# SegoleneMartin/transductive-CLIP

Hardware: AMD Instinct MI355X
Metric: transductive tasks/sec (75-query EM-Dirichlet) (higher is better)
Workload: dtype f32

## Files before the change

transductive-clip_amd/csrc/tclip_kernels.hip:

```cpp
#include <hip/hip_runtime.h>
#include <stdint.h>
#include <stdio.h>
#include <stdlib.h>
#include <string.h>

#include <algorithm>
#include <mutex>
#include <utility>
#include <vector>

#include "../../include/tclip.h"
#include "tclip_device.h"
#include "tclip_pk.h"
#include "tclip_selftest_inputs.h"

namespace tclip {

constexpr int kG64MinK = 897;

__global__ void k_log_features(const float* __restrict__ x, float* __restrict__ out, size_t n, int32_t* __restrict__ nonfinite) {
    bool bad = false;
    for (size_t i = (size_t)blockIdx.x * blockDim.x + threadIdx.x; i < n; i += (size_t)gridDim.x * blockDim.x) {
        const float v = log_f32(x[i] + kEpsF);
        out[i] = v;
// ... 976 lines not shown
        pending = st;
    }
    if (E / 2 > 0) finish(E / 2 - 1, pending);
    if (E & 1) {
        constexpr int e = E - 1;
        const float a = beta[e];
        const int i = (int)(slot[e >> 1] & 0xffffu);
        const float nb = mm_update_algebra(a, y_of(e), psi_s, my1[i], my0[i]);
        const bool ok = elem_of<E, G>(e, lane) < K;
        if (measure && ok) {
            const double df = (double)nb - (double)a;
            num += df * df;
            den += (double)a * (double)a;
        }
        beta[e] = ok ? nb : 0.0f;
    }
}

__device__ __forceinline__ void wave_lds_handoff() {
    __builtin_amdgcn_fence(__ATOMIC_RELEASE, "wavefront");
    __builtin_amdgcn_wave_barrier();
    __builtin_amdgcn_fence(__ATOMIC_ACQUIRE, "wavefront");
}

template <int E>
struct SplitPlacement {
    uint32_t slot[(E + 1) / 2];
    int nA, nB, nC;
    bool valid;
    int sorts;
};

template <int E, int G, int KC>
__device__ __forceinline__ void split_place(const float (&beta)[E], int K, int lane, float* my0, SplitPlacement<E>& pl) {
    constexpr int kFirstRagged = first_ragged_register<E, G, KC>();
    int nA = 0, nC = 0, nV = kFirstRagged * 64;
#pragma unroll
    for (int e = 0; e < E; e++) {
        float x1 = beta[e] + 1.0f;
        asm volatile("" : "+v"(x1));
        unsigned long long mA = __builtin_amdgcn_ballot_w64(x1 < 2.3f), mC = __builtin_amdgcn_ballot_w64(x1 >= 10.0f);
        if (e >= kFirstRagged) {
            const bool in_row = elem_of<E, G>(e, lane) < K;
            const unsigned long long mv = __builtin_amdgcn_ballot_w64(in_row);
            mA &= mv;
            mC &= mv;
            nV += __popcll(mv);
        }
        nA += __popcll(mA);
        nC += __popcll(mC);
    }
    const int nB = nV - nA - nC;
    int cA = 0, cB = nA, cC = nA + nB;
#pragma unroll
    for (int e = 0; e < E; e++) {
        float x1 = beta[e] + 1.0f;
        asm volatile("" : "+v"(x1));
        const bool lt = x1 < 2.3f, ge = x1 >= 10.0f;
        unsigned long long mA = __builtin_amdgcn_ballot_w64(lt), mC = __builtin_amdgcn_ballot_w64(ge);
        unsigned long long mB = ~(mA | mC);
        bool in_row = true;
        if (e >= kFirstRagged) {
            in_row = elem_of<E, G>(e, lane) < K;
            const unsigned long long mv = __builtin_amdgcn_ballot_w64(in_row);
            mA &= mv;
            mC &= mv;
            mB &= mv;
        }
        const int iA = (int)__builtin_amdgcn_mbcnt_hi((unsigned)(mA >> 32), __builtin_amdgcn_mbcnt_lo((unsigned)mA, (unsigned)cA));
        const int iB = (int)__builtin_amdgcn_mbcnt_hi((unsigned)(mB >> 32), __builtin_amdgcn_mbcnt_lo((unsigned)mB, (unsigned)cB));
        const int iC = (int)__builtin_amdgcn_mbcnt_hi((unsigned)(mC >> 32), __builtin_amdgcn_mbcnt_lo((unsigned)mC, (unsigned)cC));
        int idx = lt ? iA : iB;
        idx = ge ? iC : idx;
        if (e >= kFirstRagged) {
            idx = in_row ? idx : 0;
            if (in_row) my0[idx] = x1;
        } else {
            my0[idx] = x1;
        }
        if (e & 1) pl.slot[e >> 1] |= (uint32_t)idx << 16;
        else pl.slot[e >> 1] = (uint32_t)idx;
        cA += __popcll(mA);
        cB += __popcll(mB);
        cC += __popcll(mC);
    }
    pl.nA = nA;
    pl.nB = nB;
    pl.nC = nC;
}

template <int E, int G, int KC>
__device__ __forceinline__ void split_scatter(const float (&beta)[E], int K, int lane, float* my0, const SplitPlacement<E>& pl) {
    constexpr int kFirstRagged = first_ragged_register<E, G, KC>();
#pragma unroll
    for (int e = 0; e < E; e++) {
        const float x1 = beta[e] + 1.0f;
        const int idx = (e & 1) ? (int)(pl.slot[e >> 1] >> 16) : (int)(pl.slot[e >> 1] & 0xffffu);
        if (e >= kFirstRagged) {
            if (elem_of<E, G>(e, lane) < K) my0[idx] = x1;
        } else {
            my0[idx] = x1;
        }
    }
}

template <int E, int G, int KC = 0>
__device__ __forceinline__ void mm_iterate_wave_split(float (&beta)[E], const RowY<E, G, kSplitYRegsMaxE>& yv, int K, int lane, bool active,
                                                      const LogTabEntry* tab, float* my0, float* my1, bool measure,
                                                      double& num, double& den, SplitPlacement<E>& pl, bool keep_placement) {
    const int lane64 = threadIdx.x & 63;
    float s = 16.0f;
    bool in_domain = true;
    if (active) {
        s = row_sum_torch<E, G, KC>(beta, K, lane);
        in_domain = lane != 0 || (fast_range_f32(s) && s <= 0x1p40f);
        uint32_t largest = 0u;
#pragma unroll
        for (int e = 0; e < E; e++) largest = max(largest, f32_bits(beta[e]));
        in_domain = in_domain & mm_fast_domain_of_max_bits(largest);
    }
    s = __shfl(s, 0, G);
    if (__builtin_expect(!__all(in_domain), 0)) {
        if (active) {
            const float psi_s = digamma_f32(s);
#pragma unroll
            for (int e = 0; e < E; e++) {
                const float nb = mm_update_generic(beta[e], yv.get(e), psi_s);
                const bool ok = elem_of<E, G>(e, lane) < K;
                if (measure && ok) {
                    const double df = (double)nb - (double)beta[e];
                    num += df * df;
                    den += (double)beta[e] * (double)beta[e];
                }
                beta[e] = ok ? nb : 0.0f;
            }
        }
        pl.valid = false;
        return;
    }
    constexpr int kFirstRagged = first_ragged_register<E, G, KC>();
    int32_t smallest = 0x7f800000;
#pragma unroll
    for (int e = 0; e < E; e++) {
        int32_t bits = (int32_t)f32_bits(beta[e]);
        if (e >= kFirstRagged) bits = elem_of<E, G>(e, lane) < K ? bits : 0x7f800000;
        smallest = bits < smallest ? bits : smallest;
    }
    const bool tiny = __builtin_amdgcn_ballot_w64(smallest <= (int32_t)0x2d2febffu) != 0ull;
    const float psi_s = digamma_pos_f32(s, tab);
    bool sort_now = !(keep_placement && pl.valid);
    for (;;) {
        if (sort_now) {
            split_place<E, G, KC>(beta, K, lane, my0, pl);
            pl.sorts++;
        } else split_scatter<E, G, KC>(beta, K, lane, my0, pl);
        const int nA = pl.nA, nB = pl.nB, nC = pl.nC;
        wave_lds_handoff();
        bool misplaced = false;
        int jA = 0;
        for (; jA + 64 < nA; jA += 128) {
            const int j = jA;
            const int i0 = j + lane64, i1 = min(i0 + 64, nA - 1);
            const f2 x{my0[i0], my0[i1]};
            if (!sort_now && __builtin_amdgcn_ballot_w64(!(fmaxf(x.x, x.y) < 2.3f)) != 0ull) { misplaced = true; break; }
            f2 xr = x, acc = pk(0.0f);
#pragma unroll
            for (int k = 0; k < 8; k++) {
                acc = acc - pk_rcp_rn(xr);
                xr = xr + pk(1.0f);
            }
            const f2 m{below10_f32(xr.x), below10_f32(xr.y)};
            acc = pk_fma(-m, pk_rcp_rn(xr), acc);
            xr = xr + m;
            const f2 psi = pk_digamma_after_rec(xr, acc, tab);
            const f2 lg = pk_lgamma_sleef_1_23(x);
            my0[i0] = lg.x;
            my1[i0] = psi.x;
            my0[i1] = lg.y;
            my1[i1] = psi.y;
        }
        for (; !misplaced && jA < nA; jA += 64) {
            const int i = min(jA + lane64, nA - 1);
            const float x = my0[i];
            if (!sort_now && __builtin_amdgcn_ballot_w64(!(x < 2.3f)) != 0ull) { misplaced = true; break; }
            float xr = x, acc = 0.0f;
#pragma unroll
            for (int k = 0; k < 8; k++) {
                acc = acc - rcp_rn_f32(xr);
                xr = xr + 1.0f;
            }
            const float m = below10_f32(xr);
            acc = __builtin_fmaf(-m, rcp_rn_f32(xr), acc);
            xr = xr + m;
            const float psi = digamma_after_rec_ge10<false>(xr, acc, tab);
            bool sure;
            float lg = lgamma_sleef_1_23_f64(x, sure);
            if (__builtin_expect(__builtin_amdgcn_ballot_w64(!sure) != 0ull, 0)) lg = sure ? lg : lgamma_sleef_05_23(x);
            my0[i] = lg;
            my1[i] = psi;
        }
        auto pass_b = [&](int i) -> bool {
            const float x = my0[i];
            if (!sort_now && __builtin_amdgcn_ballot_w64(!(x >= 2.3f)) != 0ull) return true;
            float xr = x, acc = 0.0f;
#pragma unroll
            for (int k = 0; k < 8; k++) {
                const float m = below10_f32(xr);
                acc = __builtin_fmaf(-m, rcp_rn_f32(xr), acc);
                xr += m;
            }
            const float psi = digamma_after_rec_ge10<false>(xr, acc, tab);
            const float lg = lgamma_big_dense(x);
            my0[i] = lg;
            my1[i] = psi;
            return false;
        };
        const int tB = nB & 63, tC = nC & 63;
        const bool merged = tB > 0 && tC > 0 && tB + tC <= 64;
        const int endB = merged ? nB - tB : nB, endC = merged ? nC - tC : nC;
        for (int j = 0; !misplaced && j < endB; j += 64) misplaced = pass_b(nA + min(j + lane64, endB - 1));
        if (merged && !misplaced) {
            const int l = min(lane64, tB + tC - 1);
            misplaced = pass_b(l < tB ? nA + endB + l : nA + nB + endC + (l - tB));
        }
        for (int j = 0; !misplaced && j < endC; j += 64) {
            const int i = nA + nB + min(j + lane64, endC - 1);
            const float x = my0[i];
            if (!sort_now && __builtin_amdgcn_ballot_w64(!(x >= 10.0f)) != 0ull) { misplaced = true; break; }
            const float psi = digamma_after_rec_ge10<true>(x, 0.0f, tab);
            const float lg = lgamma_gt7_dense(x);
            my0[i] = lg;
            my1[i] = psi;
        }
        if (!misplaced) break;
        sort_now = true;
        wave_lds_handoff();
    }
    pl.valid = true;
    wave_lds_handoff();
    if (__builtin_expect(measure, 0)) {
        if (tiny) split_apply_updates<E, G, true, true>(beta, yv, K, lane, psi_s, my0, my1, pl.slot, num, den);
        else split_apply_updates<E, G, false, true>(beta, yv, K, lane, psi_s, my0, my1, pl.slot, num, den);
    } else if (__builtin_expect(tiny, 0)) split_apply_updates<E, G, true, false>(beta, yv, K, lane, psi_s, my0, my1, pl.slot, num, den);
    else split_apply_updates<E, G, false, false>(beta, yv, K, lane, psi_s, my0, my1, pl.slot, num, den);
    wave_lds_handoff();
}

template <int E, int G, int KC = 0>
__global__ __launch_bounds__(64, (E > 16 ? kMMWavesLarge : kMMWavesSmall)) void k_mm_split(MMArgs a) {
    static_assert(E <= kSplitMaxE, "LDS: two words per element");
    __shared__ LogTabEntry tab[16];
    __shared__ float plane0[64 * E];
    __shared__ float plane1[64 * E];
    load_log_table(tab);
    const int lane = threadIdx.x & (G - 1);
    const int group = threadIdx.x / G;
    constexpr int kRows = 64 / G;
    const int n = *a.n_rows;
    const int K = KC > 0 ? KC : a.K;
    for (int first = blockIdx.x * kRows; first < n; first += gridDim.x * kRows) {
        const int i = first + group;
        int row = i < n ? a.rows[i] : 0;
        if constexpr (G == 64) row = __builtin_amdgcn_readfirstlane(row);
        const bool active = i < n && !a.stop[row / a.rows_per_batch];
        if (!__any(active)) continue;
        float beta[E];
        RowY<E, G, kSplitYRegsMaxE> yv;
        double num = 0.0, den = 0.0;
        yv.load(a.y + (size_t)row * K, lane, K);
#pragma unroll
        for (int e = 0; e < E; e++) {
            const int d = elem_of<E, G>(e, lane);
            beta[e] = (active && d < K) ? a.alpha[(size_t)row * K + d] : 0.0f;
        }
        SplitPlacement<E> pl;
        pl.valid = false;
        pl.sorts = 0;
        for (int l = a.l0; l <= a.l1; l++)
            mm_iterate_wave_split<E, G, KC>(beta, yv, K, lane, active, tab, plane0, plane1, a.has_check && l == a.l1, num, den, pl,
                                            a.keep_placement != 0);
        if (a.work_counter && (threadIdx.x & 63) == 0) {
            atomicAdd(a.work_counter + 1, (unsigned long long)(a.l1 - a.l0 + 1));
            atomicAdd(a.work_counter + 2, (unsigned long long)pl.sorts);
        }
        if (!active) continue;
#pragma unroll
        for (int e = 0; e < E; e++) {
            const int d = elem_of<E, G>(e, lane);
            if (d < K) a.alpha[(size_t)row * K + d] = beta[e];
        }
        if (a.work_counter && lane == 0)
            atomicAdd(a.work_counter, (unsigned long long)K * (unsigned long long)(a.l1 - a.l0 + 1));
        if (a.has_check) {
            const double sn = group_sum_f64_g<G>(num), sd = group_sum_f64_g<G>(den);
            if (lane == 0) {
                a.rowpart[2 * (size_t)row] = sn;
                a.rowpart[2 * (size_t)row + 1] = sd;
            }
        }
    }
}

constexpr int kReuseQueue = 768;
struct ReuseState {
    int nS, nL;
    bool full;
    int evaluated;
};

template <int E, int G, bool kTiny, bool kMeasure>
__device__ __forceinline__ void reuse_apply_updates(float (&beta)[E], const RowY<E, G, kSplitYRegsMaxE>& yv, int K, int lane, float psi_s,
                                                    float* my0, const float* my1, uint16_t* q, int cap, ReuseState& rs,
                                                    double& num, double& den) {
    constexpr bool measure = kMeasure;
    constexpr bool kYLocal = !RowY<E, G, kSplitYRegsMaxE>::kInRegs;
    float yl[kYLocal ? E : 1];
    if constexpr (kYLocal) yv.fetch_all(yl);
    auto y_of = [&](int e) { if constexpr (kYLocal) return yl[e]; else return yv.get(e); };
    const int n_full = full_registers<E, G>(K);
    const int lane64 = threadIdx.x & 63;
    float* h0 = my0 + lane64;
    const float* h1 = my1 + lane64;
    int cS = 0, cL = 0;
    auto note = [&](int e, float a, float nb) {
        const float xo = a + 1.0f, xn = nb + 1.0f;
        const bool dirty = xn != xo, small = xn < 2.3f;
        const unsigned long long mD = __builtin_amdgcn_ballot_w64(dirty), mSm = __builtin_amdgcn_ballot_w64(small);
        const unsigned long long mS = mD & mSm, mL = mD & ~mSm;
        const int rank = lanes_below(mS);
        if (dirty) h0[64 * e] = xn;
        uint16_t* qs = q + cS;
        if (dirty && small && rank < cap - cS) qs[rank] = (uint16_t)(64 * e + lane64);
        if (__builtin_expect(mL != 0ull, 0)) {
            const int rankL = lanes_below(mL);
            if (dirty && !small && rankL < cap - cL) q[cap - 1 - cL - rankL] = (uint16_t)(64 * e + lane64);
        }
        cS += __popcll(mS);
        cL += __popcll(mL);
    };
    auto finish = [&](int p, const PkUpdateStage& st) {
        const int e = 2 * p;
        const f2 a{beta[e], beta[e + 1]};
        const f2 nb = pk_mm_update_stage2(st);
        const bool full = e + 1 < n_full;
        const bool ok0 = full || elem_of<E, G>(e, lane) < K, ok1 = full || elem_of<E, G>(e + 1, lane) < K;
        if (measure) {
            const double d0 = (double)nb.x - (double)a.x, d1 = (double)nb.y - (double)a.y;
            if (ok0) { num += d0 * d0; den += (double)a.x * (double)a.x; }
            if (ok1) { num += d1 * d1; den += (double)a.y * (double)a.y; }
        }
        if (full) {
            beta[e] = nb.x;
            beta[e + 1] = nb.y;
        } else {
            beta[e] = ok0 ? nb.x : 0.0f;
            beta[e + 1] = ok1 ? nb.y : 0.0f;
        }
        note(e, a.x, beta[e]);
        note(e + 1, a.y, beta[e + 1]);
    };
    PkUpdateStage pending;
#pragma unroll
    for (int p = 0; p < E / 2; p++) {
        const int e = 2 * p;
        const f2 a{beta[e], beta[e + 1]};
        const PkUpdateStage st = pk_mm_update_stage1_given<kTiny>(a, f2{y_of(e), y_of(e + 1)}, psi_s, h1[64 * e], h1[64 * (e + 1)],
                                                                  h0[64 * e], h0[64 * (e + 1)]);
        if (p > 0) finish(p - 1, pending);
        pending = st;
    }
    if (E / 2 > 0) finish(E / 2 - 1, pending);
    if (E & 1) {
        constexpr int e = E - 1;
        const float a = beta[e];
        const float nb = mm_update_algebra(a, y_of(e), psi_s, h1[64 * e], h0[64 * e]);
        const bool ok = elem_of<E, G>(e, lane) < K;
        if (measure && ok) {
            const double df = (double)nb - (double)a;
            num += df * df;
            den += (double)a * (double)a;
        }
        beta[e] = ok ? nb : 0.0f;
        note(e, a, beta[e]);
    }
    rs.nS = cS;
    rs.nL = cL;
    rs.full = cS + cL > cap;
}

template <int E, int G, int KC = 0>
__device__ __forceinline__ void mm_iterate_wave_reuse(float (&beta)[E], const RowY<E, G, kSplitYRegsMaxE>& yv, int K, int lane, bool active,
                                                      const LogTabEntry* tab, float* my0, float* my1, uint16_t* q, int cap, bool measure,
                                                      double& num, double& den, ReuseState& rs) {
    const int lane64 = threadIdx.x & 63;
    float s = 16.0f;
    bool in_domain = true;
    if (active) {
        s = row_sum_torch<E, G, KC>(beta, K, lane);
        in_domain = lane != 0 || (fast_range_f32(s) && s <= 0x1p40f);
        uint32_t largest = 0u;
#pragma unroll
        for (int e = 0; e < E; e++) largest = max(largest, f32_bits(beta[e]));
        in_domain = in_domain & mm_fast_domain_of_max_bits(largest);
    }
    s = __shfl(s, 0, G);
    if (__builtin_expect(!__all(in_domain), 0)) {
        if (active) {
            const float psi_s = digamma_f32(s);
#pragma unroll
            for (int e = 0; e < E; e++) {
                const float nb = mm_update_generic(beta[e], yv.get(e), psi_s);
                const bool ok = elem_of<E, G>(e, lane) < K;
                if (measure && ok) {
                    const double df = (double)nb - (double)beta[e];
                    num += df * df;
                    den += (double)beta[e] * (double)beta[e];
                }
                beta[e] = ok ? nb : 0.0f;
            }
        }
        rs.full = true;
        return;
    }
    constexpr int kFirstRagged = first_ragged_register<E, G, KC>();
    int32_t smallest = 0x7f800000;
#pragma unroll
    for (int e = 0; e < E; e++) {
        int32_t bits = (int32_t)f32_bits(beta[e]);
        if (e >= kFirstRagged) bits = elem_of<E, G>(e, lane) < K ? bits : 0x7f800000;
        smallest = bits < smallest ? bits : smallest;
    }
    const bool tiny = __builtin_amdgcn_ballot_w64(smallest <= (int32_t)0x2d2febffu) != 0ull;
    const float psi_s = digamma_pos_f32(s, tab);
    if (rs.full) {
#pragma unroll
        for (int e = 0; e < E; e++) my0[64 * e + lane64] = beta[e] + 1.0f;
        wave_lds_handoff();
#pragma unroll 1
        for (int i = lane64; i < 64 * E; i += 64) {
            const float x = my0[i];
            const bool small = x < 2.3f;
            float xr = x, acc = 0.0f;
#pragma unroll
            for (int k = 0; k < 9; k++) {
                const float m = below10_f32(xr);
                acc = __builtin_fmaf(-m, rcp_rn_f32(xr), acc);
                xr += m;
            }
            const float psi = digamma_after_rec_ge10<false>(xr, acc, tab);
            const unsigned long long m_big = __builtin_amdgcn_ballot_w64(!small);
            float lg = 0.0f;
            if (m_big != ~0ull) {
                bool sure;
                lg = lgamma_sleef_1_23_f64(small ? x : 2.0f, sure);
                if (__builtin_expect(__builtin_amdgcn_ballot_w64(!sure) != 0ull, 0)) lg = sure ? lg : lgamma_sleef_05_23(small ? x : 2.0f);
            }
            if (m_big != 0ull) {
                const float lg_big = lgamma_big_dense(small ? 8.0f : x);
                lg = small ? lg : lg_big;
            }
            my0[i] = lg;
            my1[i] = psi;
        }
        rs.evaluated += __popcll(__builtin_amdgcn_ballot_w64(active && lane == 0)) * K;
    } else {
        const int nS = rs.nS, nL = rs.nL;
        int jS = 0;
        for (; jS + 64 < nS; jS += 128) {
            const int j0 = jS + lane64, j1 = min(j0 + 64, nS - 1);
            const int i0 = q[j0], i1 = q[j1];
            const f2 x{my0[i0], my0[i1]};
            f2 xr = x, acc = pk(0.0f);
#pragma unroll
            for (int k = 0; k < 8; k++) {
                acc = acc - pk_rcp_rn(xr);
                xr = xr + pk(1.0f);
            }
            const f2 m{below10_f32(xr.x), below10_f32(xr.y)};
            acc = pk_fma(-m, pk_rcp_rn(xr), acc);
            xr = xr + m;
            const f2 psi = pk_digamma_after_rec(xr, acc, tab);
            const f2 lg = pk_lgamma_sleef_1_23(x);
            my0[i0] = lg.x;
            my1[i0] = psi.x;
            my0[i1] = lg.y;
            my1[i1] = psi.y;
        }
        for (; jS < nS; jS += 64) {
            const int i = q[min(jS + lane64, nS - 1)];
            const float x = my0[i];
            float xr = x, acc = 0.0f;
#pragma unroll
            for (int k = 0; k < 8; k++) {
                acc = acc - rcp_rn_f32(xr);
                xr = xr + 1.0f;
            }
            const float m = below10_f32(xr);
            acc = __builtin_fmaf(-m, rcp_rn_f32(xr), acc);
            xr = xr + m;
            const float psi = digamma_after_rec_ge10<false>(xr, acc, tab);
            bool sure;
            float lg = lgamma_sleef_1_23_f64(x, sure);
            if (__builtin_expect(__builtin_amdgcn_ballot_w64(!sure) != 0ull, 0)) lg = sure ? lg : lgamma_sleef_05_23(x);
            my0[i] = lg;
            my1[i] = psi;
        }
        for (int jL = 0; jL < nL; jL += 64) {
            const int i = q[cap - 1 - min(jL + lane64, nL - 1)];
            const float x = my0[i];
            float xr = x, acc = 0.0f;
#pragma unroll
            for (int k = 0; k < 8; k++) {
                const float m = below10_f32(xr);
                acc = __builtin_fmaf(-m, rcp_rn_f32(xr), acc);
                xr += m;
            }
            const float psi = digamma_after_rec_ge10<false>(xr, acc, tab);
            const float lg = lgamma_big_dense(x);
            my0[i] = lg;
            my1[i] = psi;
        }
        rs.evaluated += nS + nL;
    }
    wave_lds_handoff();
    if (__builtin_expect(measure, 0)) {
        if (tiny) reuse_apply_updates<E, G, true, true>(beta, yv, K, lane, psi_s, my0, my1, q, cap, rs, num, den);
        else reuse_apply_updates<E, G, false, true>(beta, yv, K, lane, psi_s, my0, my1, q, cap, rs, num, den);
    } else if (__builtin_expect(tiny, 0)) reuse_apply_updates<E, G, true, false>(beta, yv, K, lane, psi_s, my0, my1, q, cap, rs, num, den);
    else reuse_apply_updates<E, G, false, false>(beta, yv, K, lane, psi_s, my0, my1, q, cap, rs, num, den);
    wave_lds_handoff();
}

template <int E, int G, int KC = 0>
__global__ __launch_bounds__(64, (E > 16 ? kMMWavesLarge : kMMWavesSmall)) void k_mm_reuse(MMArgs a) {
    static_assert(E <= kSplitMaxE, "LDS: two words per element");
    constexpr int kQ = kReuseQueue < 64 * E ? kReuseQueue : 64 * E;
    __shared__ LogTabEntry tab[16];
    __shared__ float plane0[64 * E];
    __shared__ float plane1[64 * E];
    __shared__ uint16_t queue[kQ];
    load_log_table(tab);
    const int lane = threadIdx.x & (G - 1);
    const int group = threadIdx.x / G;
    constexpr int kRows = 64 / G;
    const int n = *a.n_rows;
    const int K = KC > 0 ? KC : a.K;
    const int cap = a.reuse_cap < kQ ? a.reuse_cap : kQ;
    for (int first = blockIdx.x * kRows; first < n; first += gridDim.x * kRows) {
        const int i = first + group;
        int row = i < n ? a.rows[i] : 0;
        if constexpr (G == 64) row = __builtin_amdgcn_readfirstlane(row);
        const bool active = i < n && !a.stop[row / a.rows_per_batch];
        if (!__any(active)) continue;
        float beta[E];
        RowY<E, G, kSplitYRegsMaxE> yv;
        double num = 0.0, den = 0.0;
        yv.load(a.y + (size_t)row * K, lane, K);
#pragma unroll
        for (int e = 0; e < E; e++) {
            const int d = elem_of<E, G>(e, lane);
            beta[e] = (active && d < K) ? a.alpha[(size_t)row * K + d] : 0.0f;
        }
        ReuseState rs;
        rs.nS = rs.nL = 0;
        rs.full = true;
        rs.evaluated = 0;
        for (int l = a.l0; l <= a.l1; l++)
            mm_iterate_wave_reuse<E, G, KC>(beta, yv, K, lane, active, tab, plane0, plane1, queue, cap, a.has_check && l == a.l1, num, den, rs);
        if (a.work_counter && (threadIdx.x & 63) == 0)
            atomicAdd(a.work_counter + 4, (unsigned long long)rs.evaluated);
        if (!active) continue;
#pragma unroll
        for (int e = 0; e < E; e++) {
            const int d = elem_of<E, G>(e, lane);
            if (d < K) a.alpha[(size_t)row * K + d] = beta[e];
        }
        if (a.work_counter && lane == 0) {
            const unsigned long long updates = (unsigned long long)K * (unsigned long long)(a.l1 - a.l0 + 1);
            atomicAdd(a.work_counter, updates);
            atomicAdd(a.work_counter + 5, updates);
        }
        if (a.has_check) {
            const double sn = group_sum_f64_g<G>(num), sd = group_sum_f64_g<G>(den);
            if (lane == 0) {
                a.rowpart[2 * (size_t)row] = sn;
                a.rowpart[2 * (size_t)row + 1] = sd;
            }
        }
    }
}

__global__ __launch_bounds__(256) void k_mm_decide_partial(const double* __restrict__ rowpart, const double* __restrict__ cache,
                                                           const uint8_t* __restrict__ live, int rows_per_batch,
                                                           int n_checks, int chunk, const int32_t* __restrict__ stop,
                                                           double* __restrict__ dpart) {
    const int b = blockIdx.y, slice = blockIdx.x, n_slices = gridDim.x;
    if (stop[b]) return;
    const int per = (rows_per_batch + n_slices - 1) / n_slices;
    const int r0 = slice * per, r1 = r0 + per < rows_per_batch ? r0 + per : rows_per_batch;
    const size_t base = (size_t)b * rows_per_batch;
    double num = 0.0, den = 0.0;
    for (int r = r0 + threadIdx.x; r < r1; r += blockDim.x) {
        const size_t row = base + r;
        if (live[row]) {
            num += rowpart[2 * row];
            den += rowpart[2 * row + 1];
        } else {
            num += cache[(row * n_checks + chunk) * 2];
            den += cache[(row * n_checks + chunk) * 2 + 1];
        }
    }
    __shared__ double sh[2][256];
    sh[0][threadIdx.x] = num;
    sh[1][threadIdx.x] = den;
    __syncthreads();
    for (int s = blockDim.x / 2; s > 0; s >>= 1) {
        if ((int)threadIdx.x < s) {
            sh[0][threadIdx.x] += sh[0][threadIdx.x + s];
            sh[1][threadIdx.x] += sh[1][threadIdx.x + s];
        }
        __syncthreads();
    }
    if (threadIdx.x == 0) {
        dpart[((size_t)b * n_slices + slice) * 2] = sh[0][0];
        dpart[((size_t)b * n_slices + slice) * 2 + 1] = sh[1][0];
    }
}

__global__ __launch_bounds__(1024) void k_mm_decide(const double* __restrict__ rowpart, const double* __restrict__ cache,
                                                    const uint8_t* __restrict__ live, int rows_per_batch, int n_checks,
                                                    int chunk, int has_check, int l1, int is_last, int iter_mm,
                                                    int32_t* __restrict__ stop, int32_t* __restrict__ mm_iters_out ,
                                                    int mm_stride, const double* __restrict__ dpart, int n_slices) {
    const int b = blockIdx.x;
    if (stop[b]) return;
    __shared__ double sh[2][1024];
    double num = 0.0, den = 0.0;
    if (has_check && dpart) {
        if ((int)threadIdx.x < n_slices) {
            num = dpart[((size_t)b * n_slices + threadIdx.x) * 2];
            den = dpart[((size_t)b * n_slices + threadIdx.x) * 2 + 1];
        }
    } else if (has_check) {
        const size_t base = (size_t)b * rows_per_batch;
        for (int r = threadIdx.x; r < rows_per_batch; r += blockDim.x) {
            const size_t row = base + r;
            if (live[row]) {
                num += rowpart[2 * row];
                den += rowpart[2 * row + 1];
            } else {
                num += cache[(row * n_checks + chunk) * 2];
                den += cache[(row * n_checks + chunk) * 2 + 1];
            }
        }
    }
    sh[0][threadIdx.x] = num;
    sh[1][threadIdx.x] = den;
    __syncthreads();
    for (int s = blockDim.x / 2; s > 0; s >>= 1) {
        if ((int)threadIdx.x < s) {
            sh[0][threadIdx.x] += sh[0][threadIdx.x + s];
            sh[1][threadIdx.x] += sh[1][threadIdx.x + s];
        }
        __syncthreads();
    }
    if (threadIdx.x == 0) {
        bool stopped = false;
        if (has_check) {
            const float nn = (float)__builtin_sqrt(sh[0][0]), dn = (float)__builtin_sqrt(sh[1][0]);
            const float crit = (nn * nn) / (dn * dn);
            if (crit < 1e-11f) {
                stop[b] = 1;
                mm_iters_out[(size_t)b * mm_stride] = l1 + 1;
                stopped = true;
            }
        }
        if (!stopped && is_last) mm_iters_out[(size_t)b * mm_stride] = iter_mm;
    }
}

template <int E>
__global__ __launch_bounds__(256) void k_row_consts(const float* __restrict__ alpha, const int32_t* __restrict__ rows,
                                                    const int32_t* __restrict__ n_rows, int K,
                                                    float* __restrict__ rowc) {
    const int lane = threadIdx.x & (kGroup - 1);
    const int groups_per_block = blockDim.x / kGroup;
    const int n = *n_rows;
    for (int i = blockIdx.x * groups_per_block + threadIdx.x / kGroup; i < n; i += gridDim.x * groups_per_block) {
        const int row = rows[i];
        float av[E], lg[E];
#pragma unroll
        for (int e = 0; e < E; e++) {
            const int d = e * kGroup + lane;
            const bool ok = d < K;
            av[e] = ok ? alpha[(size_t)row * K + d] : 0.0f;
            lg[e] = ok ? lgamma_f32(av[e]) : 0.0f;
        }
        const float l1 = lgamma_f32(group_sum_torch<E>(av, K, lane));
        const float l2 = -group_sum_torch<E>(lg, K, lane);
        if (lane == 0) rowc[row] = l1 + l2;
    }
}

constexpr int logits_full_regs(int E) {
    constexpr int sizes[] = {0, 1, 2, 3, 4, 6, 8, 10, 13, 16, 20, 24, 28, 32};
    int prev = 0;
    for (int s : sizes) {
        if (s >= E) break;
        prev = s;
    }
    return prev;
}
template <int E, int R>
__global__ __launch_bounds__(256) void k_logits(const float* __restrict__ alpha, const float* __restrict__ logz,
                                                const float* __restrict__ rowc, const int32_t* __restrict__ rows,
                                                const int32_t* __restrict__ n_rows, int Q, int K,
                                                float* __restrict__ logit0, const int32_t* __restrict__ only_if) {
    if (only_if && *only_if == 0) return;
    constexpr int kFull = logits_full_regs(E);
    constexpr int kGroups = 256 / kGroup;
    const int lane = threadIdx.x & (kGroup - 1);
    const int group = threadIdx.x / kGroup;
    const int n = *n_rows;
    const int nseg = (n + R - 1) / R, per_xcd = (nseg + 7) >> 3;
    const int xcd = blockIdx.x & 7;
    for (int j = blockIdx.x >> 3; j < per_xcd; j += gridDim.x >> 3) {
        const int seg = xcd * per_xcd + j;
        if (seg >= nseg) break;
        int row[R], task[R];
        bool same = true;
        float am1[R][E], rc[R];
#pragma unroll
        for (int r = 0; r < R; r++) {
            row[r] = __builtin_amdgcn_readfirstlane(rows[seg * R + r < n ? seg * R + r : seg * R]);
            task[r] = row[r] / K;
            same = same && task[r] == task[0];
            const float* ar = alpha + (size_t)row[r] * K + lane;
#pragma unroll
            for (int e = 0; e < E; e++) {
                if (e < kFull) am1[r][e] = ar[e * kGroup] - 1.0f;
                else am1[r][e] = e * kGroup + lane < K ? ar[e * kGroup] - 1.0f : 0.0f;
            }
            rc[r] = rowc[row[r]];
        }
        auto sweep = [&](int t, auto&& use) {
            for (int q = group; q < Q; q += kGroups) {
                const float* lz = logz + ((size_t)t * Q + q) * K + lane;
                float lv[E];
#pragma unroll
                for (int e = 0; e < E; e++) {
                    if (e < kFull) lv[e] = lz[e * kGroup];
                    else lv[e] = lz[e * kGroup + lane < K ? e * kGroup : K - 1 - lane];
                }
                use(q, lv);
            }
        };
        auto one = [&](int r, int t, int q, const float (&lv)[E]) {
            float pr[E];
#pragma unroll
            for (int e = 0; e < E; e++) {
                pr[e] = am1[r][e] * lv[e];
                if (e >= kFull) pr[e] = e * kGroup + lane < K ? pr[e] : 0.0f;
            }
            const float l3 = group_sum_torch<E, true, kFull>(pr, K, lane);
            if (lane == 0) logit0[((size_t)t * Q + q) * K + (row[r] - t * K)] = rc[r] + l3;
        };
        if (same) {
            sweep(task[0], [&](int q, const float (&lv)[E]) {
#pragma unroll
                for (int r = 0; r < R; r++) one(r, task[0], q, lv);
            });
        } else {
#pragma unroll
            for (int r = 0; r < R; r++) sweep(task[r], [&](int q, const float (&lv)[E]) { one(r, task[r], q, lv); });
        }
    }
}

template <int E, int kRowsPerBlock>
__global__ __launch_bounds__(256) void k_kmeans_logits_rows(const float* __restrict__ w, const float* __restrict__ z,
                                                            const uint8_t* __restrict__ need, int Q, int K, float pre,
                                                            float temperature, float* __restrict__ logit0) {
    const int lane = threadIdx.x & (kGroup - 1);
    const int group = threadIdx.x / kGroup, groups_per_block = blockDim.x / kGroup;
    const int t = blockIdx.y, k0 = blockIdx.x * kRowsPerBlock;
    bool want[kRowsPerBlock];
    bool any = false;
    float wv[kRowsPerBlock][E];
#pragma unroll
    for (int j = 0; j < kRowsPerBlock; j++) {
        want[j] = k0 + j < K && need[(size_t)t * K + k0 + j];
        any = any || want[j];
#pragma unroll
        for (int e = 0; e < E; e++) {
            const int d = e * kGroup + lane;
            wv[j][e] = (want[j] && d < K) ? w[((size_t)t * K + k0 + j) * K + d] : 0.0f;
        }
    }
    if (!any) return;
    for (int q = group; q < Q; q += groups_per_block) {
        const float* zq = z + ((size_t)t * Q + q) * K;
        float zv[E];
#pragma unroll
        for (int e = 0; e < E; e++) {
            const int d = e * kGroup + lane;
            zv[e] = zq[d < K ? d : K - 1];
        }
#pragma unroll
        for (int e = 0; e < E; e++) zv[e] = e * kGroup + lane < K ? zv[e] : 0.0f;
#pragma unroll
        for (int j = 0; j < kRowsPerBlock; j++) {
            if (!want[j]) continue;
            float pr[E];
#pragma unroll
            for (int e = 0; e < E; e++) {
                const float df = e * kGroup + lane < K ? wv[j][e] - zv[e] : 0.0f;
                pr[e] = df * df;
            }
            const float ssum = group_sum_torch<E>(pr, K, lane);
            if (lane == 0) logit0[((size_t)t * Q + q) * K + k0 + j] = temperature * (pre * ssum);
        }
    }
}

constexpr int kKmeansTile = 64;
constexpr int kKmeansTileThreads = 1024;
__global__ __launch_bounds__(kKmeansTileThreads) void k_kmeans_logits_tile(const float* __restrict__ w, const float* __restrict__ z,
                                                            const uint8_t* __restrict__ need, int Q, int K, int stride, float pre,
                                                            float temperature, float* __restrict__ logit0) {
    extern __shared__ float wt[];
    const int t = blockIdx.y, k0 = blockIdx.x * kKmeansTile;
    const int lane = threadIdx.x & 63;
    const int wave = __builtin_amdgcn_readfirstlane(threadIdx.x >> 6), n_waves = blockDim.x >> 6;
    const int k = k0 + lane;
    const bool ok = k < K && need[(size_t)t * K + k];
    if (!__syncthreads_or(ok)) return;
    const int rows = K - k0 < kKmeansTile ? K - k0 : kKmeansTile;
    const float* wsrc = w + ((size_t)t * K + k0) * K;
    {
        const int n = rows * K, step = blockDim.x;
        const int pad = stride - K;
        for (int i0 = threadIdx.x; i0 < n; i0 += 8 * step) {
            float v[8];
#pragma unroll
            for (int j = 0; j < 8; j++) v[j] = i0 + j * step < n ? wsrc[i0 + j * step] : 0.0f;
#pragma unroll
            for (int j = 0; j < 8; j++) {
                const int i = i0 + j * step;
                if (i < n) wt[i + (pad ? i / K : 0)] = v[j];
            }
        }
    }
    __syncthreads();
    const float* wl = wt + (lane < rows ? lane : rows - 1) * stride;
    const int vec_size = K >> 3, size_ilp = vec_size >> 2, nleft = vec_size - 4 * size_ilp, ntail = K - 8 * vec_size;
    for (int q = wave; q < Q; q += n_waves) {
        const float* zq = z + ((size_t)t * Q + q) * K;
        float acc[32];
#pragma unroll
        for (int sl = 0; sl < 32; sl++) acc[sl] = 0.0f;
        float zc[32];
#pragma unroll
        for (int sl = 0; sl < 32; sl++) zc[sl] = zq[sl];
        for (int m = 0; m < size_ilp; m++) {
            float zn[32];
            const int nx = m + 1 < size_ilp ? 32 * (m + 1) : 32 * m;
#pragma unroll
// ... 2213 lines not shown
```

Baseline: 165.2.

## Unify dirty-index queue and defer large-argument classification to evaluation pass

The update pass now records every changed element in a single dirty queue with one ballot, rather than splitting small and large arguments into two queues with two ballots and extra rank computations. The evaluation pass handles both the full and partial cases through one packed loop that compacts large-argument indices into a reused list and processes them in a later dense pass, flushing when the list overflows. This moves per-update branching and ballot work out of the hot update loop and uses the packed small-argument path for the full case too. In exchange it adds a flush/retry loop, reuses the queue memory for the large list, and adds LDS slack plus extra handoffs.

```diff
diff --git a/transductive-clip_amd/csrc/tclip_kernels.hip b/transductive-clip_amd/csrc/tclip_kernels.hip
--- a/transductive-clip_amd/csrc/tclip_kernels.hip
+++ b/transductive-clip_amd/csrc/tclip_kernels.hip
@@ -1302,8 +1302,9 @@
 }
 
 constexpr int kReuseQueue = 768;
+constexpr int kReuseSlack = 64;
 struct ReuseState {
-    int nS, nL;
+    int nD;
     bool full;
     int evaluated;
 };
@@ -1321,22 +1322,19 @@
     const int lane64 = threadIdx.x & 63;
     float* h0 = my0 + lane64;
     const float* h1 = my1 + lane64;
-    int cS = 0, cL = 0;
+    int cD = 0;
     auto note = [&](int e, float a, float nb) {
         const float xo = a + 1.0f, xn = nb + 1.0f;
-        const bool dirty = xn != xo, small = xn < 2.3f;
-        const unsigned long long mD = __builtin_amdgcn_ballot_w64(dirty), mSm = __builtin_amdgcn_ballot_w64(small);
-        const unsigned long long mS = mD & mSm, mL = mD & ~mSm;
-        const int rank = lanes_below(mS);
-        if (dirty) h0[64 * e] = xn;
-        uint16_t* qs = q + cS;
-        if (dirty && small && rank < cap - cS) qs[rank] = (uint16_t)(64 * e + lane64);
-        if (__builtin_expect(mL != 0ull, 0)) {
-            const int rankL = lanes_below(mL);
-            if (dirty && !small && rankL < cap - cL) q[cap - 1 - cL - rankL] = (uint16_t)(64 * e + lane64);
-        }
-        cS += __popcll(mS);
-        cL += __popcll(mL);
+        const bool dirty = xn != xo;
+        const unsigned long long mD = __builtin_amdgcn_ballot_w64(dirty);
+        int base = 2 * min(cD, cap);
+        asm("" : "+s"(base));
+        uint16_t* qs = (uint16_t*)((char*)q + base);
+        if (__builtin_expect(dirty, 1)) {
+            h0[64 * e] = xn;
+            qs[lanes_below(mD)] = (uint16_t)(64 * e + lane64);
+        }
+        cD += __popcll(mD);
     };
     auto finish = [&](int p, const PkUpdateStage& st) {
         const int e = 2 * p;
@@ -1383,9 +1381,8 @@
         beta[e] = ok ? nb : 0.0f;
         note(e, a, beta[e]);
     }
-    rs.nS = cS;
-    rs.nL = cL;
-    rs.full = cS + cL > cap;
+    rs.nD = cD;
+    rs.full = cD > cap;
 }
 
 template <int E, int G, int KC = 0>
@@ -1432,45 +1429,38 @@
     }
     const bool tiny = __builtin_amdgcn_ballot_w64(smallest <= (int32_t)0x2d2febffu) != 0ull;
     const float psi_s = digamma_pos_f32(s, tab);
-    if (rs.full) {
+    const bool full = rs.full;
+    const int n = full ? 64 * E : rs.nD;
+    if (full) {
 #pragma unroll
         for (int e = 0; e < E; e++) my0[64 * e + lane64] = beta[e] + 1.0f;
         wave_lds_handoff();
-#pragma unroll 1
-        for (int i = lane64; i < 64 * E; i += 64) {
-            const float x = my0[i];
-            const bool small = x < 2.3f;
-            float xr = x, acc = 0.0f;
-#pragma unroll
-            for (int k = 0; k < 9; k++) {
-                const float m = below10_f32(xr);
-                acc = __builtin_fmaf(-m, rcp_rn_f32(xr), acc);
-                xr += m;
-            }
-            const float psi = digamma_after_rec_ge10<false>(xr, acc, tab);
-            const unsigned long long m_big = __builtin_amdgcn_ballot_w64(!small);
-            float lg = 0.0f;
-            if (m_big != ~0ull) {
-                bool sure;
-                lg = lgamma_sleef_1_23_f64(small ? x : 2.0f, sure);
-                if (__builtin_expect(__builtin_amdgcn_ballot_w64(!sure) != 0ull, 0)) lg = sure ? lg : lgamma_sleef_05_23(small ? x : 2.0f);
-            }
-            if (m_big != 0ull) {
-                const float lg_big = lgamma_big_dense(small ? 8.0f : x);
-                lg = small ? lg : lg_big;
-            }
-            my0[i] = lg;
-            my1[i] = psi;
-        }
-        rs.evaluated += __popcll(__builtin_amdgcn_ballot_w64(active && lane == 0)) * K;
-    } else {
-        const int nS = rs.nS, nL = rs.nL;
-        int jS = 0;
-        for (; jS + 64 < nS; jS += 128) {
-            const int j0 = jS + lane64, j1 = min(j0 + 64, nS - 1);
-            const int i0 = q[j0], i1 = q[j1];
+    }
+    const int list_cap = cap + kReuseSlack;
+    int jS = 0, nL = 0;
+    for (;;) {
+        bool flush = false;
+        for (; jS + 64 < n; jS += 128) {
+            const int j0 = jS + lane64, j1 = min(j0 + 64, n - 1);
+            int i0 = j0, i1 = j1;
+            if (!full) { i0 = q[j0]; i1 = q[j1]; }
             const f2 x{my0[i0], my0[i1]};
-            f2 xr = x, acc = pk(0.0f);
+            f2 xe = x;
+            bool st0 = true, st1 = true;
+            if (__builtin_expect(__builtin_amdgcn_ballot_w64(!(fmaxf(x.x, x.y) < 2.3f)) != 0ull, 0)) {
+                const bool l0 = !(x.x < 2.3f), l1 = !(x.y < 2.3f);
+                const bool own1 = l1 && j0 + 64 < n;
+                const unsigned long long m0 = __builtin_amdgcn_ballot_w64(l0), m1 = __builtin_amdgcn_ballot_w64(own1);
+                const int c0 = __popcll(m0), c1 = __popcll(m1);
+                if (nL + c0 + c1 > list_cap) { flush = true; break; }
+                if (l0) q[nL + lanes_below(m0)] = (uint16_t)i0;
+                if (own1) q[nL + c0 + lanes_below(m1)] = (uint16_t)i1;
+                nL += c0 + c1;
+                xe = f2{l0 ? 2.0f : x.x, l1 ? 2.0f : x.y};
+                st0 = !l0;
+                st1 = !l1;
+            }
+            f2 xr = xe, acc = pk(0.0f);
 #pragma unroll
             for (int k = 0; k < 8; k++) {
                 acc = acc - pk_rcp_rn(xr);
@@ -1480,16 +1470,35 @@
             acc = pk_fma(-m, pk_rcp_rn(xr), acc);
             xr = xr + m;
             const f2 psi = pk_digamma_after_rec(xr, acc, tab);
-            const f2 lg = pk_lgamma_sleef_1_23(x);
-            my0[i0] = lg.x;
-            my1[i0] = psi.x;
-            my0[i1] = lg.y;
-            my1[i1] = psi.y;
-        }
-        for (; jS < nS; jS += 64) {
-            const int i = q[min(jS + lane64, nS - 1)];
+            const f2 lg = pk_lgamma_sleef_1_23(xe);
+            if (st0) {
+                my0[i0] = lg.x;
+                my1[i0] = psi.x;
+            }
+            if (st1) {
+                my0[i1] = lg.y;
+                my1[i1] = psi.y;
+            }
+        }
+        for (; !flush && jS < n; jS += 64) {
+            const int j = min(jS + lane64, n - 1);
+            int i = j;
+            if (!full) i = q[j];
             const float x = my0[i];
-            float xr = x, acc = 0.0f;
+            float xe = x;
+            bool st = true;
+            if (__builtin_expect(__builtin_amdgcn_ballot_w64(!(x < 2.3f)) != 0ull, 0)) {
+                const bool l = !(x < 2.3f);
+                const bool own = l && jS + lane64 < n;
+                const unsigned long long ml = __builtin_amdgcn_ballot_w64(own);
+                const int c = __popcll(ml);
+                if (nL + c > list_cap) { flush = true; break; }
+                if (own) q[nL + lanes_below(ml)] = (uint16_t)i;
+                nL += c;
+                xe = l ? 2.0f : x;
+                st = !l;
+            }
+            float xr = xe, acc = 0.0f;
 #pragma unroll
             for (int k = 0; k < 8; k++) {
                 acc = acc - rcp_rn_f32(xr);
@@ -1500,13 +1509,16 @@
             xr = xr + m;
             const float psi = digamma_after_rec_ge10<false>(xr, acc, tab);
             bool sure;
-            float lg = lgamma_sleef_1_23_f64(x, sure);
-            if (__builtin_expect(__builtin_amdgcn_ballot_w64(!sure) != 0ull, 0)) lg = sure ? lg : lgamma_sleef_05_23(x);
-            my0[i] = lg;
-            my1[i] = psi;
-        }
+            float lg = lgamma_sleef_1_23_f64(xe, sure);
+            if (__builtin_expect(__builtin_amdgcn_ballot_w64(!sure) != 0ull, 0)) lg = sure ? lg : lgamma_sleef_05_23(xe);
+            if (st) {
+                my0[i] = lg;
+                my1[i] = psi;
+            }
+        }
+        wave_lds_handoff();
         for (int jL = 0; jL < nL; jL += 64) {
-            const int i = q[cap - 1 - min(jL + lane64, nL - 1)];
+            const int i = q[min(jL + lane64, nL - 1)];
             const float x = my0[i];
             float xr = x, acc = 0.0f;
 #pragma unroll
@@ -1520,8 +1532,11 @@
             my0[i] = lg;
             my1[i] = psi;
         }
-        rs.evaluated += nS + nL;
-    }
+        if (__builtin_expect(!flush, 1)) break;
+        nL = 0;
+        wave_lds_handoff();
+    }
+    rs.evaluated += full ? __popcll(__builtin_amdgcn_ballot_w64(active && lane == 0)) * K : n;
     wave_lds_handoff();
     if (__builtin_expect(measure, 0)) {
         if (tiny) reuse_apply_updates<E, G, true, true>(beta, yv, K, lane, psi_s, my0, my1, q, cap, rs, num, den);
@@ -1538,7 +1553,7 @@
     __shared__ LogTabEntry tab[16];
     __shared__ float plane0[64 * E];
     __shared__ float plane1[64 * E];
-    __shared__ uint16_t queue[kQ];
+    __shared__ uint16_t queue[kQ + kReuseSlack];
     load_log_table(tab);
     const int lane = threadIdx.x & (G - 1);
     const int group = threadIdx.x / G;
@@ -1562,7 +1577,7 @@
             beta[e] = (active && d < K) ? a.alpha[(size_t)row * K + d] : 0.0f;
         }
         ReuseState rs;
-        rs.nS = rs.nL = 0;
+        rs.nD = 0;
         rs.full = true;
         rs.evaluated = 0;
         for (int l = a.l0; l <= a.l1; l++)
```

Measured after the change: 165.7 (median of 6 runs). About the same (+0.3%).
